# leok7v/sqz

Measured on AMD Instinct MI355X. Metric: encode MB/s + decode MB/s, 32KB window, batched blocks, 1/2/4/8 MI355X, higher is better.
Workload: dtype u8; 1 GPU; 4096 x 262144 B Zipf(s=1) byte blocks, window 2^15, one independent stream per block (BASELINE.json configs[2]); total_blocks=4096, blocks_per_gpu=4096, block_bytes=262144, win_bits=15, parallelism=1 rank; the N>1 runs shard this same batch (strong scaling), finder=index, device=AMD Radeon Graphics (gfx950:sramecc+:xnack-)

## Files before the change

### sqz_amd/csrc/lz77_index.hip

```cpp
#include "sqz_device.h"
#include "sqz_kernels.h"

namespace sqzk {

constexpr int kSharedGiveUp = 8;
constexpr int kXcds = 8;
constexpr int kSortThreads = 1024;
constexpr int kSortWaves = kSortThreads / kWave;

constexpr int kSortTile = 4 * kSortThreads;

constexpr int kSortBins = 1024;
constexpr int kSortCntRow = kSortBins + 2;
struct SortLds {
    uint32_t elem[kSortTile];
    uint16_t dig[kSortTile];
    uint16_t cnt[kSortWaves][kSortCntRow];
    uint32_t gbase[3][kSortBins];
    uint32_t delta[kSortBins];
    uint32_t wtot[kSortWaves];
};

struct __attribute__((packed)) U32u { uint32_t v; };

__device__ __forceinline__ uint32_t load_u32_unaligned(const uint8_t* p) {
    return reinterpret_cast<const U32u*>(p)->v;
}

__device__ __forceinline__ uint64_t peers_of(uint32_t digit, bool valid, int bits) {
    const uint64_t all = __ballot(valid);
    uint32_t lo = (uint32_t)all, hi = (uint32_t)(all >> 32);
#pragma unroll
    for (int bit = 0; bit < 10; bit++) {
        if (bit < bits) {
            const uint32_t mine = (uint32_t)((int32_t)(digit << (31 - bit)) >> 31);
            const uint64_t m = __ballot(mine != 0u);
            lo &= ~((uint32_t)m ^ mine);
            hi &= ~((uint32_t)(m >> 32) ^ mine);
        }
    }
    return ((uint64_t)hi << 32) | lo;
}

__device__ __forceinline__ uint32_t lanes_below(uint64_t mask) {
    return __builtin_amdgcn_mbcnt_hi((uint32_t)(mask >> 32),
                                     __builtin_amdgcn_mbcnt_lo((uint32_t)mask, 0u));
}

__device__ __forceinline__ uint32_t sort_key(const uint8_t* src, uint64_t bytes, uint32_t k) {
    return (uint64_t)k + 4 <= bytes ? (__builtin_bswap32(load_u32_unaligned(src + k)) >> 8)
                                    : (((uint32_t)src[k] << 16) | ((uint32_t)src[k + 1] << 8) | (uint32_t)src[k + 2]);
}

typedef uint32_t __attribute__((may_alias)) SortCntPair;

struct SortSec {
#ifdef SQZ_STATS
    uint64_t t[8] = {0, 0, 0, 0, 0, 0, 0, 0};
    uint64_t last = 0;
#endif
};
#ifdef SQZ_STATS
#define SORT_SEC(s, k) { const uint64_t n_ = __builtin_readcyclecounter(); (s).t[k] += n_ - (s).last; (s).last = n_; }
#define SORT_SEC_LOADS(s, k) { asm volatile("s_waitcnt vmcnt(0)" ::: "memory"); SORT_SEC(s, k) }
#else
#define SORT_SEC(s, k)
#define SORT_SEC_LOADS(s, k)
#endif

template <int kBits, bool kSmall>
__device__ __forceinline__ void sort_pass(SortLds& lds, const int pass, const uint8_t* __restrict__ src,
                                          const uint64_t bytes, const uint32_t count, const bool carry,
                                          const uint32_t* __restrict__ from, uint32_t* __restrict__ to, SortSec& sec) {
    constexpr int kDigits = 1 << kBits;
    constexpr int kTpd = kSortThreads / kDigits;
    constexpr int kWpt = kSortWaves / kTpd;
    const int tid = threadIdx.x;
    const int lane = tid & (kWave - 1);
    const int wave = __builtin_amdgcn_readfirstlane(tid >> 6);
    const bool first = kSmall ? kBits == 10 : pass == 0;
    uint32_t* const gbase = lds.gbase[pass];

    auto fetch = [&](uint32_t tile, uint32_t (&raw)[4]) {
#pragma unroll
        for (int j = 0; j < 4; j++) {
            const uint32_t k = tile + (uint32_t)(wave * 256 + j * kWave + lane);
            if (first) {
                const uint32_t last = (uint32_t)(bytes - 4);
                raw[j] = load_u32_unaligned(src + (k < last ? k : last));
            } else {
                raw[j] = from[k < count ? k : count - 1u];
            }
        }
    };
    auto key_from = [&](uint32_t raw, uint32_t k) {
        const uint32_t be = __builtin_bswap32(raw);
        return (uint64_t)k + 4 <= bytes ? be >> 8 : be & 0x00FFFFFFu;
    };
    auto decode = [&](uint32_t tile, const uint32_t (&raw)[4], uint32_t (&elem)[4], uint32_t (&digit)[4], bool (&valid)[4]) {
#pragma unroll
        for (int j = 0; j < 4; j++) {
            const uint32_t k = tile + (uint32_t)(wave * 256 + j * kWave + lane);
            valid[j] = k < count;
            const uint32_t pos = valid[j] ? (first ? k : raw[j]) : 0u;
            digit[j] = 0; elem[j] = pos;
            if (!valid[j]) { continue; }
            if (kSmall) {
                if (first) {
                    const uint32_t key = key_from(raw[j], k);
                    digit[j] = key & 0x3FFu;
                    elem[j] = pos | ((key >> 10) << 18);
                } else if (pass == 1) {
                    digit[j] = (pos >> 18) & 0x7Fu;
                } else {
                    digit[j] = pos >> 25;
                    elem[j] = pos & 0x3FFFFu;
                }
            } else if (first) {
                digit[j] = key_from(raw[j], k) & 0xFFu;
            } else if (pass == 1) {
                const uint32_t w = (uint32_t)src[pos] | ((uint32_t)src[pos + 1] << 8);
                digit[j] = w >> 8;
                if (carry) { elem[j] = pos | ((w & 0xFFu) << 24); }
            } else {
                digit[j] = carry ? (pos >> 24) : (uint32_t)src[pos];
                if (carry) { elem[j] = pos & 0x00FFFFFFu; }
            }
        }
    };

    uint32_t ahead[4], elem[4], digit[4], wrank[4];
    bool valid[4];
    fetch(0u, ahead);
    decode(0u, ahead, elem, digit, valid);
    SORT_SEC_LOADS(sec, 1)
    for (uint32_t tile = 0; tile < count; tile += (uint32_t)kSortTile) {
        const uint32_t n_tile = count - tile < (uint32_t)kSortTile ? count - tile : (uint32_t)kSortTile;
        fetch(tile + (uint32_t)kSortTile, ahead);
        {
            SortCntPair* const row = reinterpret_cast<SortCntPair*>(lds.cnt[wave]);
            for (int d = lane; d < kDigits / 2; d += kWave) { row[d] = 0u; }
        }
#pragma unroll
        for (int j = 0; j < 4; j++) {
            const uint64_t peers = peers_of(digit[j], valid[j], kBits);
            const uint32_t rank = lanes_below(peers);
            wrank[j] = valid[j] ? (uint32_t)lds.cnt[wave][digit[j]] + rank : 0u;
            __builtin_amdgcn_wave_barrier();
            if (valid[j] && rank == 0) {
                lds.cnt[wave][digit[j]] = (uint16_t)(lds.cnt[wave][digit[j]] + (uint32_t)__builtin_popcountll(peers));
            }
            __builtin_amdgcn_wave_barrier();
        }
        lds_barrier();
        SORT_SEC(sec, 2)
        const int sd = tid / kTpd;
        const int sw = (tid % kTpd) * kWpt;
        uint32_t c[kWpt], sum = 0;
#pragma unroll
        for (int i = 0; i < kWpt; i++) { c[i] = lds.cnt[sw + i][sd]; sum += c[i]; }
        const uint32_t incl = wave_scan(sum);
        if (lane == kWave - 1) { lds.wtot[wave] = incl; }
        lds_barrier();
        SORT_SEC(sec, 3)
        uint32_t at = wave_scan(lane < wave ? lds.wtot[lane] : 0u);
        at = (uint32_t)__builtin_amdgcn_readlane((int)at, kWave - 1) + incl - sum;
        const uint32_t run = at;
#pragma unroll
        for (int i = 0; i < kWpt; i++) { lds.cnt[sw + i][sd] = (uint16_t)at; at += c[i]; }
        const uint32_t run_end = kTpd > 1 ? (uint32_t)__shfl((int)at, lane | (kTpd - 1)) : at;
        if (tid % kTpd == 0) {
            const uint32_t g = gbase[sd];
            lds.delta[sd] = g - run;
            gbase[sd] = g + (run_end - run);
        }
        lds_barrier();
        SORT_SEC(sec, 4)
#pragma unroll
        for (int j = 0; j < 4; j++) {
            if (valid[j]) {
                const uint32_t slot = (uint32_t)lds.cnt[wave][digit[j]] + wrank[j];
                if (slot < (uint32_t)kSortTile) {
                    lds.elem[slot] = elem[j];
                    lds.dig[slot] = (uint16_t)digit[j];
                }
            }
        }
        lds_barrier();
        SORT_SEC(sec, 5)
#pragma unroll
        for (int j = 0; j < 4; j++) {
            const uint32_t slot = (uint32_t)(j * kSortThreads + tid);
            const uint32_t s = slot < n_tile ? slot : n_tile - 1u;
            const uint32_t dest = s + lds.delta[lds.dig[s]];
            to[dest < count ? dest : count - 1u] = lds.elem[s];
        }
        SORT_SEC(sec, 6)
        decode(tile + (uint32_t)kSortTile, ahead, elem, digit, valid);
        SORT_SEC_LOADS(sec, 1)
    }
    __threadfence_block();
    __syncthreads();
}

__global__ __launch_bounds__(kSortThreads)
void index_sort_kernel(const uint8_t* __restrict__ in,
                       const uint64_t* __restrict__ in_off,
                       uint32_t n_blocks,
                       uint32_t* __restrict__ buf_a,
                       uint32_t* __restrict__ buf_b,
                       uint64_t slots) {
    __shared__ SortLds lds;
    const uint32_t b = blockIdx.x;
    if (b >= n_blocks || in_off[b + 1] > slots) { return; }
    const int tid = threadIdx.x;
    const int lane = tid & (kWave - 1);
    const int wave = __builtin_amdgcn_readfirstlane(tid >> 6);

    const uint8_t* src = in + in_off[b];
    const uint64_t bytes = in_off[b + 1] - in_off[b];
    if (bytes < 3) { return; }
    const uint32_t count = (uint32_t)(bytes - 2);
    uint32_t* const pa = buf_a + in_off[b];
    uint32_t* const pb = buf_b + in_off[b];
    if (bytes == 3) {
        if (tid == 0) { pa[0] = 0u; }
        return;
    }
    const bool small = bytes <= (1u << 18);
    const bool carry = bytes <= (1u << 24);
    const int w0 = small ? 10 : 8, w1 = small ? 7 : 8, w2 = small ? 7 : 8;
    const int s1 = w0, s2 = w0 + w1;
    const uint32_t m0 = (1u << w0) - 1u, m1 = (1u << w1) - 1u;
    SortSec sec;
#ifdef SQZ_STATS
    sec.last = __builtin_readcyclecounter();
    const uint64_t sec_begin = sec.last;
#endif
    for (int d = tid; d < 3 * kSortBins; d += kSortThreads) { (&lds.gbase[0][0])[d] = 0; }
    __syncthreads();
    auto count_key = [&](uint32_t key) {
        atomicAdd(&lds.gbase[0][key & m0], 1u);
        atomicAdd(&lds.gbase[1][(key >> s1) & m1], 1u);
        atomicAdd(&lds.gbase[2][key >> s2], 1u);
    };
    const uint32_t quads = bytes >= 8 ? (uint32_t)((bytes - 8) / 4) + 1u : 0u;
    if ((uint32_t)tid < quads) {
        uint32_t lo = load_u32_unaligned(src + 4u * (uint32_t)tid), hi = load_u32_unaligned(src + 4u * (uint32_t)tid + 4u);
        for (uint32_t q = (uint32_t)tid; q < quads; q += (uint32_t)kSortThreads) {
            const uint64_t eight = ((uint64_t)hi << 32) | lo;
            const uint32_t nq = q + (uint32_t)kSortThreads < quads ? q + (uint32_t)kSortThreads : q;
            lo = load_u32_unaligned(src + 4u * nq); hi = load_u32_unaligned(src + 4u * nq + 4u);
#pragma unroll
            for (int j = 0; j < 4; j++) { count_key(__builtin_bswap32((uint32_t)(eight >> (8 * j))) >> 8); }
        }
    }
    for (uint32_t k = 4u * quads + (uint32_t)tid; k < count; k += (uint32_t)kSortThreads) { count_key(sort_key(src, bytes, k)); }
    __syncthreads();
    if (wave < 3) {
        uint32_t* const g = lds.gbase[wave];
        const int per = (1 << (wave == 0 ? w0 : wave == 1 ? w1 : w2)) / kWave;
        uint32_t sum = 0;
        for (int j = 0; j < per; j++) { sum += g[per * lane + j]; }
        uint32_t excl = wave_scan(sum) - sum;
        for (int j = 0; j < per; j++) { const uint32_t v = g[per * lane + j]; g[per * lane + j] = excl; excl += v; }
    }
    __syncthreads();
    SORT_SEC(sec, 0)

    if (small) {
        sort_pass<10, true>(lds, 0, src, bytes, count, carry, pb, pa, sec);
        for (int pass = 1; pass < 3; pass++) {
            sort_pass<7, true>(lds, pass, src, bytes, count, carry, pass == 1 ? pa : pb, pass == 1 ? pb : pa, sec);
        }
    } else {
        for (int pass = 0; pass < 3; pass++) {
            sort_pass<8, false>(lds, pass, src, bytes, count, carry, pass == 1 ? pa : pb, pass == 1 ? pb : pa, sec);
        }
    }
#ifdef SQZ_STATS
    if (tid == 0 && b == 1) {
        printf("sort block 1: cycles %llu: hist %llu; tiles: loads %llu rank %llu scan_a %llu scan_b %llu place %llu copy_out %llu\n",
               (unsigned long long)(sec.last - sec_begin), (unsigned long long)sec.t[0], (unsigned long long)sec.t[1],
               (unsigned long long)sec.t[2], (unsigned long long)sec.t[3], (unsigned long long)sec.t[4],
               (unsigned long long)sec.t[5], (unsigned long long)sec.t[6]);
    }
#endif
}

__global__ __launch_bounds__(256)
void index_match_kernel(const uint8_t* __restrict__ in,
                        const uint64_t* __restrict__ in_off,
                        uint32_t n_blocks, uint32_t window,
                        const uint32_t* __restrict__ sorted,
                        uint32_t* __restrict__ match, uint32_t groups, uint64_t slots) {
    const uint32_t xcd = blockIdx.x % (uint32_t)kXcds;
    const uint32_t local = blockIdx.x / (uint32_t)kXcds;
    const uint32_t b = (local / groups) * (uint32_t)kXcds + xcd;
    const uint32_t group = local % groups;
    if (b >= n_blocks || in_off[b + 1] > slots) { return; }
    const uint8_t* src = in + in_off[b];
    const uint64_t bytes = in_off[b + 1] - in_off[b];
    if (bytes < 3) { return; }
    const uint32_t n = (uint32_t)bytes;
    const uint32_t count = n - 2;
    const uint32_t* S = sorted + in_off[b];
    uint32_t* M = match + in_off[b];

    const int lane = (int)(threadIdx.x & (kWave - 1));
    const uint32_t pages = (count + (uint32_t)kWave - 1u) / (uint32_t)kWave;
    const uint32_t waves = groups * (blockDim.x / (uint32_t)kWave);
    const uint32_t per_wave = (pages + waves - 1u) / waves;
    const uint32_t wave_id = group * (blockDim.x / (uint32_t)kWave) + (threadIdx.x - (uint32_t)lane) / (uint32_t)kWave;
    const uint32_t page_lo = wave_id * per_wave;
    const uint32_t page_hi = page_lo + per_wave < pages ? page_lo + per_wave : pages;
    auto load16 = [&](uint32_t at, uint32_t& w0, uint32_t& w1, uint32_t& w2, uint32_t& w3) {
        if (at + 16 <= n) {
            w0 = load_u32_unaligned(src + at); w1 = load_u32_unaligned(src + at + 4);
            w2 = load_u32_unaligned(src + at + 8); w3 = load_u32_unaligned(src + at + 12);
        } else {
            uint32_t w[4] = {0, 0, 0, 0};
            for (uint32_t k = 0; k < 16 && at + k < n; k++) { w[k >> 2] |= (uint32_t)src[at + k] << (8 * (k & 3)); }
            w0 = w[0]; w1 = w[1]; w2 = w[2]; w3 = w[3];
        }
    };
    uint32_t prev_i = 0, prev0 = 0, prev1 = 0, prev2 = 0, prev3 = 0;
    if (page_lo > 0 && page_lo < page_hi) {
        prev_i = S[(page_lo - 1u) * (uint32_t)kWave + (uint32_t)lane];
        load16(prev_i, prev0, prev1, prev2, prev3);
    }
    for (uint32_t pg = page_lo; pg < page_hi; pg++) {
        const uint32_t r0 = pg * (uint32_t)kWave;
        const bool have_prev = pg > 0;
        const uint32_t r = r0 + (uint32_t)lane;
        const bool valid = r < count;
        const uint32_t i = valid ? S[r] : 0u;
        const uint32_t cap = (n - i) < (uint32_t)kLenMax ? (n - i) : (uint32_t)kLenMax;
        const uint32_t reach = i < window - 1 ? i : window - 1;
        uint32_t own0 = 0, own1 = 0, own2 = 0, own3 = 0;
        if (valid) { load16(i, own0, own1, own2, own3); }
        const uint32_t key = own0 & 0x00FFFFFFu;
        uint32_t best = 0, dist = 0;
        auto walk = [&](uint32_t q_from) {
            if (q_from == 0 || best >= cap) { return; }
            auto inside = [&](uint32_t r) {
                const uint32_t p = S[r];
                if (p + 4 > n) { return false; }
                return (load_u32_unaligned(src + p) & 0x00FFFFFFu) == key && i - p <= reach;
            };
            uint32_t q_lo;
            {
                uint32_t d = 4, bad = 0, good = q_from;
                bool open = true;
                while (open) {
                    if (d >= q_from) { bad = 0; open = false; if (inside(0)) { good = 0; } else { bad = 1; } }
                    else if (inside(q_from - d)) { good = q_from - d; d <<= 1; }
                    else { bad = q_from - d + 1; open = false; }
                }
                uint32_t lo = bad, hi = good;
                while (lo < hi) {
                    const uint32_t mid = lo + ((hi - lo) >> 1);
                    if (inside(mid)) { hi = mid; } else { lo = mid + 1; }
                }
                q_lo = lo;
            }
            uint8_t own_next = best >= (uint32_t)kLenMin ? src[i + best] : (uint8_t)0;
            for (uint32_t q = q_from; q > q_lo && best < cap; ) {
                q--;
                const uint32_t p = S[q];
                if (best >= (uint32_t)kLenMin && src[p + best] != own_next) { continue; }
                uint32_t k = 3;
                while (k < cap) {
                    if (i + k + 4 <= n) {
                        const uint32_t x = load_u32_unaligned(src + p + k) ^ load_u32_unaligned(src + i + k);
                        if (x != 0) { k += (uint32_t)__builtin_ctz(x) >> 3; break; }
                        k += 4;
                    } else {
                        if (src[p + k] != src[i + k]) { break; }
                        k++;
                    }
                }
                if (k > cap) { k = cap; }
                if (k > best) {
                    best = k; dist = i - p;
                    if (best < cap) { own_next = src[i + best]; }
                }
            }
        };
        const uint32_t key0 = (uint32_t)__builtin_amdgcn_readfirstlane((int)key);
        if (__ballot(valid && key == key0 && i + 16 <= n) == ~0ull) {
            bool done = false, deferred = false;
            uint32_t resume = 0;
            uint32_t page_base = r0, page = i, pb0 = own0, pb1 = own1, pb2 = own2, pb3 = own3;
            for (int64_t c = (int64_t)r0 + kWave - 2; c >= 0; c--) {
                if (c < (int64_t)page_base) {
                    page_base -= (uint32_t)kWave;
                    page = S[page_base + (uint32_t)lane];
                    load16(page, pb0, pb1, pb2, pb3);
                }
                const int at = (int)(c - (int64_t)page_base);
                const uint32_t pc = (uint32_t)__builtin_amdgcn_readlane((int)page, at);
                const bool below = (int64_t)r > c;
                const uint32_t d = i - pc;
                if (below && d > reach) { done = true; }
                if (__ballot(!done) == 0) { break; }
                const uint32_t c0 = (uint32_t)__builtin_amdgcn_readlane((int)pb0, at);
                if ((c0 & 0x00FFFFFFu) != key0) { break; }
                const uint32_t c1 = (uint32_t)__builtin_amdgcn_readlane((int)pb1, at);
                const uint32_t c2 = (uint32_t)__builtin_amdgcn_readlane((int)pb2, at);
                const uint32_t c3 = (uint32_t)__builtin_amdgcn_readlane((int)pb3, at);
                const uint32_t x0 = own0 ^ c0, x1 = own1 ^ c1, x2 = own2 ^ c2, x3 = own3 ^ c3;
                uint32_t len = x0 != 0 ? ((uint32_t)__builtin_ctz(x0) >> 3)
                             : x1 != 0 ? 4u + ((uint32_t)__builtin_ctz(x1) >> 3)
                             : x2 != 0 ? 8u + ((uint32_t)__builtin_ctz(x2) >> 3)
                             : x3 != 0 ? 12u + ((uint32_t)__builtin_ctz(x3) >> 3) : 16u;
                const bool want = below && !done;
                if (want && len == 16u && cap > 16u) {
                    deferred = true;
                    resume = (uint32_t)c + 1u;
                    done = true;
                } else {
                    if (len > cap) { len = cap; }
                    if (want && len > best) {
                        best = len; dist = d;
                        if (best >= cap) { done = true; }
                    }
                }
                if (__builtin_popcountll(__ballot(deferred)) >= kSharedGiveUp) {
                    if (!done) {
                        deferred = true;
                        resume = below ? (uint32_t)c : r;
                        done = true;
                    }
                    break;
                }
            }
            if (deferred) { walk(resume); }
            M[i] = best >= (uint32_t)kLenMin ? ((best << 16) | dist) : (key & 0xFFu);
            prev_i = i; prev0 = own0; prev1 = own1; prev2 = own2; prev3 = own3;
            continue;
        }
        bool done = !valid;
        bool later = false;
        uint32_t resume = 0;
        for (int k = 1; k <= kWave; k++) {
            const int from = lane - k;
            const bool in_cur = from >= 0;
            if (!done && !in_cur && !have_prev) { done = true; }
            if (__ballot(!done) == 0) { break; }
            const int addr = (from & (kWave - 1)) << 2;
            uint32_t pc = (uint32_t)__builtin_amdgcn_ds_bpermute(addr, (int)i);
            uint32_t c0 = (uint32_t)__builtin_amdgcn_ds_bpermute(addr, (int)own0);
            uint32_t c1 = (uint32_t)__builtin_amdgcn_ds_bpermute(addr, (int)own1);
            const bool back = __ballot(!done && !in_cur) != 0;
            if (back) {
                const uint32_t qc = (uint32_t)__builtin_amdgcn_ds_bpermute(addr, (int)prev_i);
                const uint32_t q0 = (uint32_t)__builtin_amdgcn_ds_bpermute(addr, (int)prev0);
                const uint32_t q1 = (uint32_t)__builtin_amdgcn_ds_bpermute(addr, (int)prev1);
                pc = in_cur ? pc : qc; c0 = in_cur ? c0 : q0; c1 = in_cur ? c1 : q1;
            }
            const uint32_t x0 = own0 ^ c0, x1 = own1 ^ c1;
            if (!done && (x0 & 0x00FFFFFFu) != 0) { done = true; }
            const uint32_t d = i - pc;
            if (!done && d > reach) { done = true; }
            uint32_t len = x0 != 0 ? ((uint32_t)__builtin_ctz(x0) >> 3) : x1 != 0 ? 4u + ((uint32_t)__builtin_ctz(x1) >> 3) : 8u;
            if (__ballot(!done && len == 8u && cap > 8u) != 0) {
                uint32_t c2 = (uint32_t)__builtin_amdgcn_ds_bpermute(addr, (int)own2);
                uint32_t c3 = (uint32_t)__builtin_amdgcn_ds_bpermute(addr, (int)own3);
                if (back) {
                    const uint32_t q2 = (uint32_t)__builtin_amdgcn_ds_bpermute(addr, (int)prev2);
                    const uint32_t q3 = (uint32_t)__builtin_amdgcn_ds_bpermute(addr, (int)prev3);
                    c2 = in_cur ? c2 : q2; c3 = in_cur ? c3 : q3;
                }
                const uint32_t x2 = own2 ^ c2, x3 = own3 ^ c3;
                if (len == 8u) {
                    len = x2 != 0 ? 8u + ((uint32_t)__builtin_ctz(x2) >> 3) : x3 != 0 ? 12u + ((uint32_t)__builtin_ctz(x3) >> 3) : 16u;
                }
            }
            if (!done) {
                if (len == 16u && cap > 16u) {
                    later = true;
                    resume = r - (uint32_t)k + 1u;
                    done = true;
                } else {
                    if (len > cap) { len = cap; }
                    if (len > best) {
                        best = len; dist = d;
                        if (best >= cap) { done = true; }
                    }
                    if (!done && k == kWave) {
                        later = true;
                        resume = r - (uint32_t)kWave;
                        done = true;
                    }
                }
            }
        }
        if (later) { walk(resume); }
        if (valid) { M[i] = best >= (uint32_t)kLenMin ? ((best << 16) | dist) : (key & 0xFFu); }
        prev_i = i; prev0 = own0; prev1 = own1; prev2 = own2; prev3 = own3;
    }
}

constexpr int kChunk = 32;
constexpr int kTile = kChunk * kWave;
constexpr int kChunkRow = kChunk + 1;

struct ParseLds {
    uint32_t m[kChunkRow * kWave];
};

__device__ __forceinline__ uint32_t parse_slot(uint32_t k) { return k + (k / (uint32_t)kChunk); }

__device__ __forceinline__ uint32_t parse_step(uint32_t w) {
    const uint32_t len = w >> 16;
    return len != 0 ? len : 1u;
}

__device__ __forceinline__ bool lazy_defers(uint32_t w, uint32_t w1) {
    const uint32_t len = w >> 16;
    return len >= (uint32_t)kLenMin && (w1 >> 16) > len;
}

constexpr int kTileRows = kTile / kWave;
__device__ __forceinline__ void parse_fetch(uint32_t (&w)[kTileRows], const uint32_t* __restrict__ M,
                                            const uint64_t tile, const uint64_t bytes, const int lane) {
    const uint64_t left = bytes - tile;
    const uint32_t last = left < (uint64_t)kTile ? (uint32_t)left - 1u : (uint32_t)kTile - 1u;
    const uint32_t* __restrict__ T = M + tile;
#pragma unroll
    for (int j = 0; j < kTileRows; j++) {
        const uint32_t k = (uint32_t)(j * kWave + lane);
        w[j] = T[k < last ? k : last];
    }
}

__device__ __forceinline__ uint32_t per_tile(uint32_t v) {
#ifndef SQZ_WAVE_EMU
    asm volatile("" : "+v"(v));
#endif
    return v;
}

struct ParseSec {
#ifdef SQZ_STATS
    uint64_t t[5] = {0, 0, 0, 0, 0};
    uint64_t last = 0;
#endif
};
#ifdef SQZ_STATS
#define PARSE_SEC(s, k) SORT_SEC(s, k)
#define PARSE_SEC_LOADS(s, k) SORT_SEC_LOADS(s, k)
#else
#define PARSE_SEC(s, k)
#define PARSE_SEC_LOADS(s, k)
#endif

template <bool kLazy>
__global__ __launch_bounds__(kWave)
void index_parse_kernel(const uint8_t* __restrict__ in,
                        const uint64_t* __restrict__ in_off,
                        uint32_t n_blocks,
                        const uint32_t* __restrict__ match,
                        uint32_t* __restrict__ tokens,
                        uint32_t* __restrict__ tok_count, uint64_t slots) {
    __shared__ ParseLds lds;
    const uint32_t b = blockIdx.x;
    if (b >= n_blocks) { return; }
    const int lane = threadIdx.x;
    if (in_off[b + 1] > slots) {
        if (lane == 0) { tok_count[b] = kRefused; }
        return;
    }
    const uint8_t* src = in + in_off[b];
    const uint64_t bytes = in_off[b + 1] - in_off[b];
    const uint32_t* M = match + in_off[b];
    uint32_t* tok = tokens + in_off[b];

    if (bytes == 0) {
        if (lane == 0) { tok_count[b] = 0; }
        return;
    }
    const uint32_t lit1 = (uint32_t)src[bytes - 1];
    const uint32_t lit2 = (uint32_t)src[bytes >= 2 ? bytes - 2 : 0];

    ParseSec sec;
#ifdef SQZ_STATS
    sec.last = __builtin_readcyclecounter();
    const uint64_t sec_begin = sec.last;
#endif
    uint32_t ntok = 0;
    uint32_t entry = 0;
    uint32_t fly[kTileRows];
    parse_fetch(fly, M, 0, bytes, lane);
    uint32_t fly_next = 0;
    auto fetch_next = [&](const uint64_t tile) __attribute__((always_inline)) {
        const uint64_t at = tile + (uint64_t)per_tile((uint32_t)kTile);
        fly_next = M[at < bytes ? at : bytes - 1];
    };
    if constexpr (kLazy) { fetch_next(0); }
    auto do_tile = [&](const uint64_t tile) __attribute__((always_inline)) -> bool {
        const uint64_t left = bytes - tile;
        const uint32_t have = left < (uint64_t)kTile ? (uint32_t)left : (uint32_t)kTile;
        if (entry >= have) { return false; }
        PARSE_SEC_LOADS(sec, 0)
        lds_barrier();
        const int t2 = left < (uint64_t)(kTile + 2) ? (int)left - 2 : kTile;
        uint32_t* const mine_at = &lds.m[parse_slot((uint32_t)lane)];
#pragma unroll
        for (int j = 0; j < kTileRows; j++) {
            const int tj = t2 - j * kWave;
            mine_at[j * (kWave + kWave / kChunk)] = lane < tj ? fly[j] : lane == tj ? lit2 : lit1;
        }
        uint32_t over = 0;
        if constexpr (kLazy) {
            over = left > (uint64_t)(kTile + 2) ? fly_next : 0u;
        }
        lds_barrier();
        const uint64_t ahead = tile + (uint64_t)kTile < bytes ? tile + (uint64_t)kTile : tile;
        parse_fetch(fly, M, ahead, bytes, lane);
        if constexpr (kLazy) { fetch_next(ahead); }
        PARSE_SEC(sec, 1)

        const uint32_t lo = (uint32_t)lane * (uint32_t)kChunk;
        const uint32_t room = have > lo ? (have - lo < (uint32_t)kChunk ? have - lo : (uint32_t)kChunk) : 0u;
        const uint32_t* row = &lds.m[lane * kChunkRow];
        uint32_t defer = 0;
        if constexpr (kLazy) {
            const uint32_t behind = lane + 1 < kWave ? lds.m[(lane + 1 < kWave ? lane + 1 : lane) * kChunkRow] : over;
            uint32_t w = row[0];
#pragma unroll 1
            for (int j0 = 0; j0 < kChunk; j0 += 8) {
#pragma unroll
                for (int j = 0; j < 8; j++) {
                    const uint32_t w1 = j0 + j + 1 < kChunk ? row[j0 + j + 1] : behind;
                    defer |= (lazy_defers(w, w1) ? 1u : 0u) << (j0 + j);
                    w = w1;
                }
            }
        }
        uint32_t guess = 0;
        uint32_t p = 0;
        while (p < room) {
            guess |= 1u << p;
            const uint32_t w = row[p];
            if constexpr (kLazy) { p += ((defer >> p) & 1u) != 0 ? 1u : parse_step(w); } else { p += parse_step(w); }
        }
        const uint32_t guess_out = lo + p;
        PARSE_SEC(sec, 2)

        uint32_t extra = 0;
        uint32_t from = (uint32_t)kChunk;
        uint32_t e = entry;
        while (e < have) {
            const uint32_t l = e / (uint32_t)kChunk;
            const uint32_t clo = l * (uint32_t)kChunk;
            const uint32_t g = (uint32_t)__builtin_amdgcn_readlane((int)guess, (int)l);
            uint32_t q = e - clo;
            if (((g >> q) & 1u) != 0) {
                e = (uint32_t)__builtin_amdgcn_readlane((int)guess_out, (int)l);
                if ((uint32_t)lane == l) { from = q; }
                continue;
            }
            const uint32_t croom = have - clo < (uint32_t)kChunk ? have - clo : (uint32_t)kChunk;
            uint32_t real = 0;
            do {
                real |= 1u << q;
                const uint32_t w = (uint32_t)__builtin_amdgcn_readfirstlane((int)lds.m[l * kChunkRow + q]);
                if constexpr (kLazy) {
                    const uint32_t dl = (uint32_t)__builtin_amdgcn_readlane((int)defer, (int)l);
                    q += ((dl >> q) & 1u) != 0 ? 1u : parse_step(w);
                } else {
                    q += parse_step(w);
                }
            } while (q < croom && ((g >> q) & 1u) == 0);
            const bool met = q < croom;
            e = met ? (uint32_t)__builtin_amdgcn_readlane((int)guess_out, (int)l) : clo + q;
            if ((uint32_t)lane == l) { extra = real; from = met ? q : (uint32_t)kChunk; }
        }
        const uint32_t mine = extra | (from < (uint32_t)kChunk ? guess & (~0u << from) : 0u);
        entry = e - (uint32_t)kTile;
        uint32_t give = 0, give_j0 = 0, give_j1 = 0, give_b0 = 0, give_b1 = 0;
        if constexpr (kLazy) {
            give = mine & defer;
            const uint32_t second = give & (give - 1u);
            give_j0 = give != 0 ? (uint32_t)__builtin_ctz(give) : 0u;
            give_j1 = second != 0 ? (uint32_t)__builtin_ctz(second) : give_j0;
            const uint64_t at0 = tile + (uint64_t)(lo + give_j0), at1 = tile + (uint64_t)(lo + give_j1);
            give_b0 = src[at0 < bytes ? at0 : bytes - 1];
            give_b1 = src[at1 < bytes ? at1 : bytes - 1];
        }
        PARSE_SEC(sec, 3)

        uint32_t mw[kChunk];
#pragma unroll
        for (int j = 0; j < kChunk; j++) { mw[j] = row[j]; }
        const uint32_t cnt = (uint32_t)__builtin_popcount(mine);
        const uint32_t incl = wave_scan(cnt);
        const uint32_t total = (uint32_t)__builtin_amdgcn_readlane((int)incl, kWave - 1);
        lds_barrier();
        uint32_t at = incl - cnt;
#pragma unroll
        for (int j = 0; j < kChunk; j++) {
            if ((mine >> j) & 1u) {
                lds.m[at++] = (mw[j] >> 16) != 0 ? (kTokMatch | mw[j]) : (mw[j] & 0xFFu);
            }
        }
        if constexpr (kLazy) {
            const uint32_t first = incl - cnt;
            auto slot_of = [&](uint32_t j) { return first + (uint32_t)__builtin_popcount(mine & ((1u << j) - 1u)); };
            uint32_t rest = give;
            if (rest != 0) { lds.m[slot_of(give_j0)] = give_b0; rest &= rest - 1u; }
            if (rest != 0) { lds.m[slot_of(give_j1)] = give_b1; rest &= rest - 1u; }
            while (rest != 0) {
                const uint32_t j = (uint32_t)__builtin_ctz(rest);
                rest &= rest - 1u;
                lds.m[slot_of(j)] = (uint32_t)src[tile + (uint64_t)(lo + j)];
            }
        }
        lds_barrier();
        uint32_t* const out = tok + ntok;
        const uint32_t last = total - 1u;
        const uint32_t ln = per_tile((uint32_t)lane);
#pragma unroll
        for (int j = 0; j < kTileRows; j++) {
            const uint32_t k = (uint32_t)(j * kWave) + ln;
            const uint32_t n = (k < last ? k : last) & (uint32_t)(kTile - 1);
            out[n] = lds.m[n];
        }
        ntok += total;
        PARSE_SEC(sec, 4)
        return true;
    };
    static_assert(kTile > kLenMax, "a token never reaches over a whole tile");
    if (do_tile(0)) {
        for (uint64_t tile = (uint64_t)kTile; tile < bytes; tile += (uint64_t)kTile) {
            if (!do_tile(tile)) { break; }
        }
    }
    if (lane == 0) { tok_count[b] = ntok; }
#ifdef SQZ_STATS
    if (lane == 0 && b == 1) {
        printf("parse block 1: cycles %llu: tiles: arrived %llu stage %llu guess %llu fixup %llu write %llu\n",
               (unsigned long long)(sec.last - sec_begin), (unsigned long long)sec.t[0], (unsigned long long)sec.t[1],
               (unsigned long long)sec.t[2], (unsigned long long)sec.t[3], (unsigned long long)sec.t[4]);
    }
#endif
}

void launch_index_sort(const uint8_t* in, const uint64_t* in_off, uint32_t n_blocks,
                       uint32_t* buf_a, uint32_t* buf_b, uint64_t slots,
                       hipStream_t stream) {
    if (n_blocks == 0) { return; }
    hipLaunchKernelGGL(index_sort_kernel, dim3(n_blocks), dim3(kSortThreads), 0, stream,
                       in, in_off, n_blocks, buf_a, buf_b, slots);
}

void launch_index_match(const uint8_t* in, const uint64_t* in_off, uint32_t n_blocks,
                        uint32_t window, const uint32_t* sorted, uint32_t* match,
                        uint32_t match_groups, uint64_t slots, hipStream_t stream) {
    if (n_blocks == 0) { return; }
    if (match_groups < 1) { match_groups = 1; }
    const uint32_t rounded = (n_blocks + (uint32_t)kXcds - 1) / (uint32_t)kXcds * (uint32_t)kXcds;
    while ((uint64_t)match_groups * rounded > 0x7FFFFFFFull) { match_groups = (match_groups + 1) / 2; }
    hipLaunchKernelGGL(index_match_kernel, dim3(rounded * match_groups), dim3(256), 0, stream,
                       in, in_off, n_blocks, window, sorted, match, match_groups, slots);
}

void launch_index_parse(const uint8_t* in, const uint64_t* in_off, uint32_t n_blocks,
                        const uint32_t* match, uint32_t* tokens, uint32_t* tok_count,
                        uint64_t slots, hipStream_t stream) {
    if (n_blocks == 0) { return; }
    hipLaunchKernelGGL(index_parse_kernel<false>, dim3(n_blocks), dim3(kWave), 0, stream,
                       in, in_off, n_blocks, match, tokens, tok_count, slots);
}

void launch_index_parse_lazy(const uint8_t* in, const uint64_t* in_off, uint32_t n_blocks,
                             const uint32_t* match, uint32_t* tokens, uint32_t* tok_count,
                             uint64_t slots, hipStream_t stream) {
    if (n_blocks == 0) { return; }
    hipLaunchKernelGGL(index_parse_kernel<true>, dim3(n_blocks), dim3(kWave), 0, stream,
                       in, in_off, n_blocks, match, tokens, tok_count, slots);
}

}
```

Measured before the change: 15130 MB/s.

## Software-pipeline position and 16-byte window loads in index match kernel

Restructures the index match kernel so that sorted positions two pages ahead and 16-byte data windows for the next page are requested before the current page is matched. The old per-byte tail fallback is replaced by a clamped vector load plus a lane-wise shift fixup. The shared-key run does the same prefetching for the page further back. Stores become unconditional, with invalid lanes rewriting lane 0's value, and optional stats instrumentation is added. This aims to hide global memory latency, at the cost of more live registers and more complex control flow.

```diff
diff --git a/sqz_amd/csrc/lz77_index.hip b/sqz_amd/csrc/lz77_index.hip
--- a/sqz_amd/csrc/lz77_index.hip
+++ b/sqz_amd/csrc/lz77_index.hip
@@ -285,6 +285,29 @@
                (unsigned long long)sec.t[2], (unsigned long long)sec.t[3], (unsigned long long)sec.t[4],
                (unsigned long long)sec.t[5], (unsigned long long)sec.t[6]);
     }
+#endif
+}
+
+struct MatchSec {
+#ifdef SQZ_STATS
+    uint64_t t[6] = {0, 0, 0, 0, 0, 0};
+    uint64_t last = 0;
+    uint32_t pages = 0, whole = 0;
+#endif
+};
+#ifdef SQZ_STATS
+#define MATCH_SEC(s, k) SORT_SEC(s, k)
+#define MATCH_SEC_LOADS(s, k) { asm volatile("s_waitcnt vmcnt(1)" ::: "memory"); SORT_SEC(s, k) }
+#else
+#define MATCH_SEC(s, k)
+#define MATCH_SEC_LOADS(s, k)
+#endif
+
+typedef uint32_t U32x4u __attribute__((vector_size(16), aligned(1), may_alias));
+
+__device__ __forceinline__ void landed(uint32_t a, uint32_t b, uint32_t c, uint32_t d, uint32_t e) {
+#if defined(__HIP_DEVICE_COMPILE__)
+    asm volatile("" :: "v"(a), "v"(b), "v"(c), "v"(d), "v"(e));
 #endif
 }
 
@@ -311,34 +334,47 @@
     const uint32_t pages = (count + (uint32_t)kWave - 1u) / (uint32_t)kWave;
     const uint32_t waves = groups * (blockDim.x / (uint32_t)kWave);
     const uint32_t per_wave = (pages + waves - 1u) / waves;
-    const uint32_t wave_id = group * (blockDim.x / (uint32_t)kWave) + (threadIdx.x - (uint32_t)lane) / (uint32_t)kWave;
+    const uint32_t wave_id = group * (blockDim.x / (uint32_t)kWave) +
+                             (uint32_t)__builtin_amdgcn_readfirstlane((int)((threadIdx.x - (uint32_t)lane) / (uint32_t)kWave));
     const uint32_t page_lo = wave_id * per_wave;
     const uint32_t page_hi = page_lo + per_wave < pages ? page_lo + per_wave : pages;
-    auto load16 = [&](uint32_t at, uint32_t& w0, uint32_t& w1, uint32_t& w2, uint32_t& w3) {
-        if (at + 16 <= n) {
-            w0 = load_u32_unaligned(src + at); w1 = load_u32_unaligned(src + at + 4);
-            w2 = load_u32_unaligned(src + at + 8); w3 = load_u32_unaligned(src + at + 12);
-        } else {
-            uint32_t w[4] = {0, 0, 0, 0};
-            for (uint32_t k = 0; k < 16 && at + k < n; k++) { w[k >> 2] |= (uint32_t)src[at + k] << (8 * (k & 3)); }
-            w0 = w[0]; w1 = w[1]; w2 = w[2]; w3 = w[3];
-        }
-    };
-    uint32_t prev_i = 0, prev0 = 0, prev1 = 0, prev2 = 0, prev3 = 0;
-    if (page_lo > 0 && page_lo < page_hi) {
-        prev_i = S[(page_lo - 1u) * (uint32_t)kWave + (uint32_t)lane];
-        load16(prev_i, prev0, prev1, prev2, prev3);
-    }
-    for (uint32_t pg = page_lo; pg < page_hi; pg++) {
+    if (page_lo >= page_hi) { return; }
+    MatchSec sec;
+#ifdef SQZ_STATS
+    sec.last = __builtin_readcyclecounter();
+    const uint64_t sec_begin = sec.last;
+#endif
+
+    auto request16 = [&](uint32_t at, uint32_t& w0, uint32_t& w1, uint32_t& w2, uint32_t& w3) {
+        const uint32_t from = at < n - 16u ? at : n - 16u;
+        const U32x4u v = *reinterpret_cast<const U32x4u*>(src + from);
+        w0 = v[0]; w1 = v[1]; w2 = v[2]; w3 = v[3];
+    };
+    auto settle16 = [&](uint32_t at, uint32_t& w0, uint32_t& w1, uint32_t& w2, uint32_t& w3) {
+        if (__ballot(at + 16u > n) == 0) { return; }
+        const uint32_t sh = at + 16u > n ? at + 16u - n : 0u;
+        if (sh & 8u) { w0 = w2; w1 = w3; w2 = 0; w3 = 0; }
+        if (sh & 4u) { w0 = w1; w1 = w2; w2 = w3; w3 = 0; }
+        const uint32_t bits = (sh & 3u) * 8u, up = (32u - bits) & 31u, keep = bits != 0 ? ~0u : 0u;
+        w0 = (w0 >> bits) | ((w1 << up) & keep);
+        w1 = (w1 >> bits) | ((w2 << up) & keep);
+        w2 = (w2 >> bits) | ((w3 << up) & keep);
+        w3 >>= bits;
+    };
+    auto request_positions = [&](uint32_t pg) {
+        const uint32_t r = (pg < page_hi ? pg : page_hi - 1u) * (uint32_t)kWave + (uint32_t)lane;
+        return S[r < count ? r : count - 1u];
+    };
+
+    auto match_page = [&](const uint32_t pg, const bool valid, const uint32_t i,
+                          const uint32_t own0, const uint32_t own1, const uint32_t own2, const uint32_t own3,
+                          const uint32_t prev_i, const uint32_t prev0, const uint32_t prev1, const uint32_t prev2,
+                          const uint32_t prev3) -> uint32_t {
         const uint32_t r0 = pg * (uint32_t)kWave;
         const bool have_prev = pg > 0;
         const uint32_t r = r0 + (uint32_t)lane;
-        const bool valid = r < count;
-        const uint32_t i = valid ? S[r] : 0u;
         const uint32_t cap = (n - i) < (uint32_t)kLenMax ? (n - i) : (uint32_t)kLenMax;
         const uint32_t reach = i < window - 1 ? i : window - 1;
-        uint32_t own0 = 0, own1 = 0, own2 = 0, own3 = 0;
-        if (valid) { load16(i, own0, own1, own2, own3); }
         const uint32_t key = own0 & 0x00FFFFFFu;
         uint32_t best = 0, dist = 0;
         auto walk = [&](uint32_t q_from) {
@@ -365,9 +401,10 @@
                 q_lo = lo;
             }
             uint8_t own_next = best >= (uint32_t)kLenMin ? src[i + best] : (uint8_t)0;
+            uint32_t p = 0;
             for (uint32_t q = q_from; q > q_lo && best < cap; ) {
                 q--;
-                const uint32_t p = S[q];
+                p = S[q];
                 if (best >= (uint32_t)kLenMin && src[p + best] != own_next) { continue; }
                 uint32_t k = 3;
                 while (k < cap) {
@@ -386,59 +423,71 @@
                     if (best < cap) { own_next = src[i + best]; }
                 }
             }
+            landed(p, own_next, p, p, p);
         };
         const uint32_t key0 = (uint32_t)__builtin_amdgcn_readfirstlane((int)key);
         if (__ballot(valid && key == key0 && i + 16 <= n) == ~0ull) {
             bool done = false, deferred = false;
             uint32_t resume = 0;
             uint32_t page_base = r0, page = i, pb0 = own0, pb1 = own1, pb2 = own2, pb3 = own3;
-            for (int64_t c = (int64_t)r0 + kWave - 2; c >= 0; c--) {
-                if (c < (int64_t)page_base) {
-                    page_base -= (uint32_t)kWave;
-                    page = S[page_base + (uint32_t)lane];
-                    load16(page, pb0, pb1, pb2, pb3);
-                }
-                const int at = (int)(c - (int64_t)page_base);
-                const uint32_t pc = (uint32_t)__builtin_amdgcn_readlane((int)page, at);
-                const bool below = (int64_t)r > c;
-                const uint32_t d = i - pc;
-                if (below && d > reach) { done = true; }
-                if (__ballot(!done) == 0) { break; }
-                const uint32_t c0 = (uint32_t)__builtin_amdgcn_readlane((int)pb0, at);
-                if ((c0 & 0x00FFFFFFu) != key0) { break; }
-                const uint32_t c1 = (uint32_t)__builtin_amdgcn_readlane((int)pb1, at);
-                const uint32_t c2 = (uint32_t)__builtin_amdgcn_readlane((int)pb2, at);
-                const uint32_t c3 = (uint32_t)__builtin_amdgcn_readlane((int)pb3, at);
-                const uint32_t x0 = own0 ^ c0, x1 = own1 ^ c1, x2 = own2 ^ c2, x3 = own3 ^ c3;
-                uint32_t len = x0 != 0 ? ((uint32_t)__builtin_ctz(x0) >> 3)
-                             : x1 != 0 ? 4u + ((uint32_t)__builtin_ctz(x1) >> 3)
-                             : x2 != 0 ? 8u + ((uint32_t)__builtin_ctz(x2) >> 3)
-                             : x3 != 0 ? 12u + ((uint32_t)__builtin_ctz(x3) >> 3) : 16u;
-                const bool want = below && !done;
-                if (want && len == 16u && cap > 16u) {
-                    deferred = true;
-                    resume = (uint32_t)c + 1u;
-                    done = true;
-                } else {
-                    if (len > cap) { len = cap; }
-                    if (want && len > best) {
-                        best = len; dist = d;
-                        if (best >= cap) { done = true; }
+            uint32_t far_i = prev_i, back_i = 0, back0 = 0, back1 = 0, back2 = 0, back3 = 0;
+            int64_t c = (int64_t)r0 + kWave - 2;
+            for (bool walking = true; walking; ) {
+                back_i = far_i;
+                far_i = S[(page_base >= 2u * (uint32_t)kWave ? page_base - 2u * (uint32_t)kWave : 0u) + (uint32_t)lane];
+                request16(back_i, back0, back1, back2, back3);
+                for (; c >= (int64_t)page_base; c--) {
+                    const int at = (int)(c - (int64_t)page_base);
+                    const uint32_t pc = (uint32_t)__builtin_amdgcn_readlane((int)page, at);
+                    const bool below = (int64_t)r > c;
+                    const uint32_t d = i - pc;
+                    if (below && d > reach) { done = true; }
+                    if (__ballot(!done) == 0) { walking = false; break; }
+                    const uint32_t c0 = (uint32_t)__builtin_amdgcn_readlane((int)pb0, at);
+                    if ((c0 & 0x00FFFFFFu) != key0) { walking = false; break; }
+                    const uint32_t c1 = (uint32_t)__builtin_amdgcn_readlane((int)pb1, at);
+                    const uint32_t c2 = (uint32_t)__builtin_amdgcn_readlane((int)pb2, at);
+                    const uint32_t c3 = (uint32_t)__builtin_amdgcn_readlane((int)pb3, at);
+                    const uint32_t x0 = own0 ^ c0, x1 = own1 ^ c1, x2 = own2 ^ c2, x3 = own3 ^ c3;
+                    uint32_t len = x0 != 0 ? ((uint32_t)__builtin_ctz(x0) >> 3)
+                                 : x1 != 0 ? 4u + ((uint32_t)__builtin_ctz(x1) >> 3)
+                                 : x2 != 0 ? 8u + ((uint32_t)__builtin_ctz(x2) >> 3)
+                                 : x3 != 0 ? 12u + ((uint32_t)__builtin_ctz(x3) >> 3) : 16u;
+                    const bool want = below && !done;
+                    if (want && len == 16u && cap > 16u) {
+                        deferred = true;
+                        resume = (uint32_t)c + 1u;
+                        done = true;
+                    } else {
+                        if (len > cap) { len = cap; }
+                        if (want && len > best) {
+                            best = len; dist = d;
+                            if (best >= cap) { done = true; }
+                        }
                     }
-                }
-                if (__builtin_popcountll(__ballot(deferred)) >= kSharedGiveUp) {
-                    if (!done) {
-                        deferred = true;
-                        resume = below ? (uint32_t)c : r;
-                        done = true;
+                    if (__builtin_popcountll(__ballot(deferred)) >= kSharedGiveUp) {
+                        if (!done) {
+                            deferred = true;
+                            resume = below ? (uint32_t)c : r;
+                            done = true;
+                        }
+                        walking = false;
+                        break;
                     }
-                    break;
-                }
-            }
+                }
+                if (!walking || page_base == 0) { break; }
+                page_base -= (uint32_t)kWave;
+                page = back_i; pb0 = back0; pb1 = back1; pb2 = back2; pb3 = back3;
+                settle16(page, pb0, pb1, pb2, pb3);
+            }
+            landed(far_i, back0, back1, back2, back3);
+#ifdef SQZ_STATS
+            sec.whole++;
+#endif
+            MATCH_SEC(sec, 4)
             if (deferred) { walk(resume); }
-            M[i] = best >= (uint32_t)kLenMin ? ((best << 16) | dist) : (key & 0xFFu);
-            prev_i = i; prev0 = own0; prev1 = own1; prev2 = own2; prev3 = own3;
-            continue;
+            MATCH_SEC(sec, 3)
+            return best >= (uint32_t)kLenMin ? ((best << 16) | dist) : (key & 0xFFu);
         }
         bool done = !valid;
         bool later = false;
@@ -452,8 +501,7 @@
             uint32_t pc = (uint32_t)__builtin_amdgcn_ds_bpermute(addr, (int)i);
             uint32_t c0 = (uint32_t)__builtin_amdgcn_ds_bpermute(addr, (int)own0);
             uint32_t c1 = (uint32_t)__builtin_amdgcn_ds_bpermute(addr, (int)own1);
-            const bool back = __ballot(!done && !in_cur) != 0;
-            if (back) {
+            if (__ballot(!done && !in_cur) != 0) {
                 const uint32_t qc = (uint32_t)__builtin_amdgcn_ds_bpermute(addr, (int)prev_i);
                 const uint32_t q0 = (uint32_t)__builtin_amdgcn_ds_bpermute(addr, (int)prev0);
                 const uint32_t q1 = (uint32_t)__builtin_amdgcn_ds_bpermute(addr, (int)prev1);
@@ -467,7 +515,7 @@
             if (__ballot(!done && len == 8u && cap > 8u) != 0) {
                 uint32_t c2 = (uint32_t)__builtin_amdgcn_ds_bpermute(addr, (int)own2);
                 uint32_t c3 = (uint32_t)__builtin_amdgcn_ds_bpermute(addr, (int)own3);
-                if (back) {
+                if (__ballot(!done && !in_cur) != 0) {
                     const uint32_t q2 = (uint32_t)__builtin_amdgcn_ds_bpermute(addr, (int)prev2);
                     const uint32_t q3 = (uint32_t)__builtin_amdgcn_ds_bpermute(addr, (int)prev3);
                     c2 = in_cur ? c2 : q2; c3 = in_cur ? c3 : q3;
@@ -496,10 +544,64 @@
                 }
             }
         }
+        MATCH_SEC(sec, 2)
         if (later) { walk(resume); }
-        if (valid) { M[i] = best >= (uint32_t)kLenMin ? ((best << 16) | dist) : (key & 0xFFu); }
+        MATCH_SEC(sec, 3)
+        return best >= (uint32_t)kLenMin ? ((best << 16) | dist) : (key & 0xFFu);
+    };
+    auto word_out = [&](bool valid, uint32_t i, uint32_t word) {
+        const uint32_t first_i = (uint32_t)__builtin_amdgcn_readlane((int)i, 0);
+        const uint32_t first_word = (uint32_t)__builtin_amdgcn_readlane((int)word, 0);
+        M[valid ? i : first_i] = valid ? word : first_word;
+        MATCH_SEC(sec, 5)
+    };
+    if (n < 16u) {
+        const bool valid = (uint32_t)lane < count;
+        const uint32_t i = valid ? S[lane] : 0u;
+        uint32_t w[4] = {0, 0, 0, 0};
+        if (valid) { for (uint32_t k = 0; k < 16 && i + k < n; k++) { w[k >> 2] |= (uint32_t)src[i + k] << (8 * (k & 3)); } }
+        word_out(valid, i, match_page(0u, valid, i, w[0], w[1], w[2], w[3], 0u, 0u, 0u, 0u, 0u));
+        return;
+    }
+    uint32_t prev_i = request_positions(page_lo > 0 ? page_lo - 1u : 0u), prev0, prev1, prev2, prev3;
+    uint32_t i = request_positions(page_lo);
+    uint32_t next_i = request_positions(page_lo + 1u);
+    MATCH_SEC_LOADS(sec, 0)
+    i = page_lo * (uint32_t)kWave + (uint32_t)lane < count ? i : 0u;
+    uint32_t own0, own1, own2, own3;
+    request16(prev_i, prev0, prev1, prev2, prev3);
+    request16(i, own0, own1, own2, own3);
+    settle16(prev_i, prev0, prev1, prev2, prev3);
+    for (uint32_t pg = page_lo; ; pg++) {
+        const bool has_next = pg + 1u < page_hi;
+        const bool valid = pg * (uint32_t)kWave + (uint32_t)lane < count;
+        const uint32_t far_i = request_positions(pg + 2u);
+        next_i = has_next && (pg + 1u) * (uint32_t)kWave + (uint32_t)lane < count ? next_i : 0u;
+        uint32_t next0, next1, next2, next3;
+        request16(next_i, next0, next1, next2, next3);
+        settle16(i, own0, own1, own2, own3);
+        if (!valid) { own0 = 0; own1 = 0; own2 = 0; own3 = 0; }
+#ifdef SQZ_STATS
+        sec.pages++;
+#endif
+        MATCH_SEC(sec, 1)
+        const uint32_t word = match_page(pg, valid, i, own0, own1, own2, own3, prev_i, prev0, prev1, prev2, prev3);
+        word_out(valid, i, word);
+        if (!has_next) { break; }
+        MATCH_SEC_LOADS(sec, 1)
         prev_i = i; prev0 = own0; prev1 = own1; prev2 = own2; prev3 = own3;
-    }
+        i = next_i; own0 = next0; own1 = next1; own2 = next2; own3 = next3;
+        next_i = far_i;
+    }
+#ifdef SQZ_STATS
+    if (lane == 0 && (wave_id == 0 || wave_id == waves / 2) && b == 1) {
+        printf("match block 1, wave %u: cycles %llu over %u pages (%u whole-run): positions %llu arrived %llu neighbours %llu "
+               "own_walk %llu shared_walk %llu store %llu\n",
+               wave_id, (unsigned long long)(sec.last - sec_begin), sec.pages, sec.whole, (unsigned long long)sec.t[0],
+               (unsigned long long)sec.t[1], (unsigned long long)sec.t[2], (unsigned long long)sec.t[3],
+               (unsigned long long)sec.t[4], (unsigned long long)sec.t[5]);
+    }
+#endif
 }
 
 constexpr int kChunk = 32;
```

New measurement: 15240 MB/s, median of 6. No clear change (+0.8%).
